# sqeazy/sqeazy

Measured on AMD Instinct MI355X. Metric: encode GB/s (input voxels) for bitswap1->lz4 uint16 volume, higher is better.
Workload: dtype u16

## Files before the change

sqeazy_amd/csrc/sqy_capi.cpp:

```cpp
#include "../../include/sqeazy_amd.h"

#include <hip/hip_runtime.h>

#include <algorithm>
#include <chrono>
#include <climits>
#include <cstdint>
#include <cstdio>
#include <cstdlib>
#include <cstring>
#include <atomic>
#include <condition_variable>
#include <memory>
#include <mutex>
#include <string>
#include <thread>
#include <vector>

#include "sqy_kernels.h"
#include "sqy_lanes.hpp"
#include "sqy_pipeline.hpp"

namespace {

// ... 23 lines not shown
        return dflt;
    }
    return (long)x;
}
constexpr long kWarmupMax = 1l << 30;
constexpr long kStageLanesDefault = 2, kParseLanesDefault = 3;
struct Options {
    std::atomic<long> transpose_chain;
    std::atomic<long> transpose_chain_caller_streams;
    std::atomic<long> block_parallel;
    std::atomic<long> block_parallel_warmup;
    std::atomic<long> block_parallel_stats;
    std::atomic<long> tail_scan;
    std::atomic<long> decode_two_waves;
    std::atomic<long> noise_digest;
    std::atomic<long> transpose_blocks_per_cu;
    std::atomic<long> stored_tail_index;
    std::atomic<long> host_l2_bytes;
    std::atomic<long> decode_frames_subset;
    std::atomic<long> decode_slabs_joint;
    std::atomic<long> stage_lanes;
    std::atomic<long> parse_lanes;
    std::atomic<long> lane_calls{0}, lane_backlog_fallbacks{0}, lane_blocked_fallbacks{0};
    std::atomic<long> call_stamps{0};
    Options()
        : transpose_chain(env_flag("SQY_NO_TRANSPOSE_CHAIN") ? 0 : 1), transpose_chain_caller_streams(env_flag("SQY_TRANSPOSE_CHAIN_CALLER_STREAMS")),
          block_parallel(env_flag("SQY_NO_BLOCK_PARALLEL") ? 0 : 1), block_parallel_warmup(env_number("SQY_BLOCK_PARALLEL_WARMUP", 65536, 0, kWarmupMax)),
          block_parallel_stats(env_flag("SQY_BLOCK_PARALLEL_STATS")), tail_scan(env_flag("SQY_NO_TAIL_SCAN") ? 0 : 1),
          decode_two_waves(env_flag("SQY_NO_DECODE_TWO_WAVES") ? 0 : 1), noise_digest(env_flag("SQY_NO_NOISE_DIGEST") ? 0 : 1),
          transpose_blocks_per_cu(env_number("SQY_TRANSPOSE_BLOCKS_PER_CU", 32, 1, 64)), stored_tail_index(env_flag("SQY_NO_STORED_TAIL_INDEX") ? 0 : 1),
          host_l2_bytes((long)sqy::host_l2_cache_bytes()), decode_frames_subset(env_flag("SQY_NO_DECODE_FRAMES_SUBSET") ? 0 : 1),
          decode_slabs_joint(env_flag("SQY_NO_DECODE_SLABS_JOINT") ? 0 : 1), stage_lanes(env_number("SQY_STAGE_LANES", kStageLanesDefault, 0, 2)),
          parse_lanes(env_number("SQY_PARSE_LANES", kParseLanesDefault, 1, sqy::LanePicker::kMaxLanes)) { sqy::set_bitswap1_blocks_per_cu(transpose_blocks_per_cu.load()); }
    std::atomic<long>* find(const char* name)
    {
        if (!name) return nullptr;
        if (!std::strcmp(name, "transpose_chain")) return &transpose_chain;
        if (!std::strcmp(name, "transpose_chain_caller_streams")) return &transpose_chain_caller_streams;
        if (!std::strcmp(name, "block_parallel")) return &block_parallel;
        if (!std::strcmp(name, "block_parallel_warmup")) return &block_parallel_warmup;
        if (!std::strcmp(name, "block_parallel_stats")) return &block_parallel_stats;
        if (!std::strcmp(name, "tail_scan")) return &tail_scan;
        if (!std::strcmp(name, "decode_two_waves")) return &decode_two_waves;
        if (!std::strcmp(name, "noise_digest")) return &noise_digest;
        if (!std::strcmp(name, "transpose_blocks_per_cu")) return &transpose_blocks_per_cu;
        if (!std::strcmp(name, "stored_tail_index")) return &stored_tail_index;
        if (!std::strcmp(name, "host_l2_bytes")) return &host_l2_bytes;
        if (!std::strcmp(name, "decode_frames_subset")) return &decode_frames_subset;
        if (!std::strcmp(name, "decode_slabs_joint")) return &decode_slabs_joint;
        if (!std::strcmp(name, "stage_lanes")) return &stage_lanes;
        if (!std::strcmp(name, "parse_lanes")) return &parse_lanes;
        if (!std::strcmp(name, "lane_calls")) return &lane_calls;
        if (!std::strcmp(name, "lane_backlog_fallbacks")) return &lane_backlog_fallbacks;
        if (!std::strcmp(name, "lane_blocked_fallbacks")) return &lane_blocked_fallbacks;
        if (!std::strcmp(name, "call_stamps")) return &call_stamps;
        return nullptr;
    }
};
Options g_opt;

struct CallStamps {
    enum { entry, lanes_taken, clear_launched, transpose_launched, parse_queued, sync_returned, returned, kStamps };
    long seq = -1;
    long lane = -1;
    long thread = 0;
    long ns[kStamps] = {};
    void stamp(int i) { ns[i] = (long)std::chrono::duration_cast<std::chrono::nanoseconds>(std::chrono::steady_clock::now().time_since_epoch()).count(); }
};
constexpr size_t kStampRing = 8192;
std::mutex g_stamps_mu;
std::vector<CallStamps> g_stamps;
size_t g_stamps_next = 0;
struct StampScope {
    CallStamps rec;
    const bool on;
    StampScope() : on(g_opt.call_stamps.load(std::memory_order_relaxed) != 0) 
    {
// ... 72 lines not shown
    } while (0)

void prof_collect(std::vector<PendingEvent>& pending)
{
    for (PendingEvent& p : pending) {
        float ms = 0;
        if (hipEventSynchronize(p.b) == hipSuccess && hipEventElapsedTime(&ms, p.a, p.b) == hipSuccess) {
            std::lock_guard<std::mutex> lock(g_prof_mu);
            size_t i = 0;
            for (; i < g_prof.size(); ++i) if (g_prof[i].name == p.name) break;
            if (i == g_prof.size()) g_prof.push_back(ProfEntry{p.name, 0, 0});
            g_prof[i].ms += ms;
            g_prof[i].launches += 1;
        }
        ev_give(p.a);
        ev_give(p.b);
    }
    pending.clear();
}

struct DevBuf {
    void* p = nullptr;
    size_t cap = 0;
    int ensure(size_t bytes, bool quiet = false)
    {
        if (bytes <= cap) return 0;
        if (p) { hipFree(p); p = nullptr; cap = 0; }
        const size_t want = (bytes + ((size_t)1 << 20) - 1) & ~(((size_t)1 << 20) - 1);
        if (hipMalloc(&p, want) != hipSuccess) {
            if (!quiet) std::fprintf(stderr, "[sqeazy]\t unable to allocate %zu bytes of HBM workspace\n", want);
            (void)hipGetLastError();
            p = nullptr;
            return 1;
        }
        cap = want;
        return 0;
    }
    void release() { if (p) hipFree(p); p = nullptr; cap = 0; }
};

struct HostBuf {
    void* p = nullptr;
    size_t cap = 0;
    int ensure(size_t bytes)
    {
        if (bytes <= cap) return 0;
        if (p) { hipHostFree(p); p = nullptr; cap = 0; }
        const size_t want = (bytes + ((size_t)1 << 16) - 1) & ~(((size_t)1 << 16) - 1);
        if (hipHostMalloc(&p, want, hipHostMallocDefault) != hipSuccess) {
            std::fprintf(stderr, "[sqeazy]\t unable to allocate %zu bytes of pinned host memory\n", want);
            (void)hipGetLastError();
            p = nullptr;
            return 1;
        }
        cap = want;
        return 0;
    }
    void release() { if (p) hipHostFree(p); p = nullptr; cap = 0; }
};

struct Workspace {
    DevBuf ping, pong, lz4_scratch, csize, frame_off, io_src, io_dst, small, plan, dedupe;
    DevBuf spec;
    DevBuf diff_side;
    DevBuf digest;
    DevBuf bkrd;
    DevBuf subset;
    DevBuf range_full;
    DevBuf slabs_index;
    DevBuf slabs_joint;
    DevBuf slabs_out;
    HostBuf slabs_host;
    void* pinned = nullptr;
    void release_buffers()
    {
        ping.release(); pong.release(); lz4_scratch.release(); csize.release(); frame_off.release();
        io_src.release(); io_dst.release(); small.release(); plan.release(); dedupe.release(); diff_side.release(); spec.release(); digest.release(); bkrd.release();
        subset.release(); range_full.release(); slabs_index.release(); slabs_joint.release(); slabs_out.release(); slabs_host.release();
    }
};

struct Stager {
    static constexpr int kLanes = 4;
    static constexpr size_t kSlice = 8u << 20;
    char* pin[kLanes][2] = {};
    hipStream_t st[kLanes] = {};
    hipEvent_t ev[kLanes][2] = {};
    bool ready = false;

    bool init()
    {
        if (ready) return true;
        for (int l = 0; l < kLanes; ++l) {
            if (hipStreamCreateWithFlags(&st[l], hipStreamNonBlocking) != hipSuccess) return false;
            for (int b = 0; b < 2; ++b) {
                if (hipHostMalloc((void**)&pin[l][b], kSlice, hipHostMallocDefault) != hipSuccess) return false;
                if (hipEventCreateWithFlags(&ev[l][b], hipEventDisableTiming) != hipSuccess) return false;
            }
// ... 239 lines not shown
    LaneLease* lanes;
    CallStamps* stamps;
    Pipeline pipe;
    std::vector<uint64_t> dims;
    uint64_t len;
    int elem_size;
    void* d_dst;
    uint64_t dst_capacity;
    long* dstoffset;
    FrameQuery* fq;

    const uint8_t* cur;
    int cur_elem;
    uint64_t cur_len;
    bool use_ping = true;

    struct {
        const uint32_t* piece_hash = nullptr;
        bool inplace = false;
        uint64_t t0 = 0, in_stride = 0;
        uint32_t* digest = nullptr;
        uint32_t digest_stride = 0;
        bool dedupe_cleared = false;
        const uint64_t* frame_map = nullptr;
        uint64_t frame_bytes = 0;
    } prep;
    struct DiffSide { const uint16_t* p = nullptr; uint32_t w = 0, X = 0; } side;
    struct {
        bool on = false;
        int block_id = 0;
        uint64_t total = 0, chunk = 0, nchunks = 0, stride = 0;
        const sqy::Lz4Block* blocks = nullptr;
        const uint32_t* dup_of = nullptr;
        uint64_t* tail_info = nullptr;
        bool inplace_done = false;
        uint64_t blob_at = 0, blob_bytes = 0, payload_bytes = 0;
    } lz4;

    EncodeCall(Context& c, hipStream_t s, Pipeline&& p, std::vector<uint64_t>&& d, uint64_t voxels, int elem, const void* src, void* dst,
               uint64_t capacity, long* offset, FrameQuery* frames, LaneLease* lane_lease, CallStamps* call_stamps)
        : cx(c), ws(&c.ws), pend(&c.pending), stream(s), lanes(lane_lease), stamps(call_stamps), pipe(std::move(p)), dims(std::move(d)), len(voxels), elem_size(elem), d_dst(dst),
          dst_capacity(capacity), dstoffset(offset), fq(frames), cur(static_cast<const uint8_t*>(src)), cur_elem(elem), cur_len(voxels) {}

    uint8_t* next_buf(size_t bytes)
    {
        DevBuf& b = use_ping ? ws->ping : ws->pong;
        use_ping = !use_ping;
        return b.ensure(bytes) ? nullptr : static_cast<uint8_t*>(b.p);
    }
    int produced(const uint8_t* out) { cur = out; return 0; }
    bool is_tail(size_t si) const { return pipe.sink_index >= 0 && (int)si > pipe.sink_index; }
    bool not_3d(const char* scheme) const
    {
        if (dims.size() != 3) std::fprintf(stderr, "[sqeazy::detail::%s::encode] received non-3D shape which is currently unsupported!\n", scheme);
        return dims.size() != 3;
    }
    bool followed_by(size_t si, StageKind k) const { return si + 1 < pipe.stages.size() && pipe.stages[si + 1].kind == k; }
    void stage_shape(size_t si, uint64_t& Z, uint64_t& Y, uint64_t& X) const
    {
        const bool flat = is_tail(si) && cur_len * (uint64_t)cur_elem != len;
        Z = flat ? 1 : dims[0]; Y = flat ? 1 : dims[1]; X = flat ? cur_len : dims[2];
    }

    int take_lanes(std::unique_lock<std::mutex>& lock)
    {
// ... 73 lines not shown
            if (words && chunked && chunk % 1024 == 0 && total > chunk) {
                const uint64_t nch = (total + chunk - 1) / chunk;
                const uint64_t ph_bytes = (words * 4 + 63) & ~(uint64_t)63;
                if (ws->dedupe.ensure(ph_bytes + sqy::lz4_dedupe_work_bytes(nch) + ((nch * 4 + 7) & ~(uint64_t)7) + sqy::lz4_holes_map_bytes(nch, (uint32_t)chunk))) return 1;
                ph = static_cast<uint32_t*>(ws->dedupe.p);
                prep.piece_hash = ph;
                if (dstoffset && si + 2 == pipe.stages.size() && (chunk & (chunk - 1)) == 0) {
                    const uint64_t hdr_max = sqy::header_pack(elem_size, false, dims, pipe.name(), (uint64_t)INT_MAX).size() + 2;
                    uint64_t t0 = hdr_max;
                    while ((reinterpret_cast<uintptr_t>(d_dst) + t0 + 11) & 15) ++t0;
                    if (t0 + nch * (chunk + 15) <= dst_capacity) {
                        gap_chunk = chunk;
                        prep.t0 = t0;
                        prep.in_stride = chunk + 15;
                        prep.inplace = true;
                        if (ws->plan.ensure((nch + 1) * sizeof(uint32_t))) return 1;
                        const uint32_t dstride = sqy::lz4_noise_digest_stride((uint32_t)chunk);
                        if (g_opt.noise_digest.load() && dstride && (cur_len / 8) % chunk == 0 && lz.accel >= 0 &&
                            !ws->digest.ensure(nch * (uint64_t)dstride * sizeof(uint32_t), true)) {
                            prep.digest = static_cast<uint32_t*>(ws->digest.p);
                            prep.digest_stride = dstride;
                        }
                        if (take_lanes(lane_lock)) return 1;
                        SQY_HIP(sqy::launch_lz4_dedupe_clear(static_cast<uint8_t*>(ws->dedupe.p) + ph_bytes, nch, static_cast<uint32_t*>(ws->plan.p), stream));
                        prep.dedupe_cleared = true;
                        if (stamps) stamps->stamp(CallStamps::clear_launched);
                    }
                }
            }
        }
        uint8_t* out = gap_chunk ? static_cast<uint8_t*>(d_dst) + prep.t0 + 11 : next_buf(cur_len * cur_elem);
        if (!out) return 1;
        if (!gap_chunk && ph && (reinterpret_cast<uintptr_t>(out) & 15)) { ph = nullptr; prep.piece_hash = nullptr; }
        const bool on_lanes = lanes && lanes->taken();
        const bool owned = stream != nullptr && stream == cx.stream;
        int devid = 0;
        const bool chain = !on_lanes && g_opt.transpose_chain.load() && (owned || g_opt.transpose_chain_caller_streams.load()) && gap_chunk &&
                           hipGetDevice(&devid) == hipSuccess && devid >= 0 && devid < kMaxDev;
        std::unique_lock<std::mutex> tlock;
        if (chain) {
            if (!cx.t_done && hipEventCreateWithFlags(&cx.t_done, hipEventDisableTiming) != hipSuccess) return 1;
            tlock = std::unique_lock<std::mutex>(g_tchain_mu[devid]);
            const auto now = std::chrono::steady_clock::now();
            if (g_tchain_last[devid] && g_tchain_last[devid] != cx.t_done && now - g_tchain_when[devid] < std::chrono::milliseconds(5))
                SQY_HIP(hipStreamWaitEvent(stream, g_tchain_last[devid], 0));
            g_tchain_when[devid] = now;
        }
// ... 303 lines not shown
                                                                   static_cast<uint32_t*>(ws->csize.p), d_redo, n_redo, stream, prep.frame_map, prep.frame_bytes,
                                                                   prep.in_stride));
        return 0;
    }

    int lz4_inplace_finish(uint32_t* d_redo, const std::string& hdr_prefix, const std::string& hdr_suffix)
    {
        const Lz4Descriptor fd = lz4_descriptor(lz4.block_id);
        uint8_t* outb = static_cast<uint8_t*>(d_dst);
        volatile uint64_t* record = static_cast<volatile uint64_t*>(ws->pinned);
        const bool fused_tail = lz4.nchunks <= 65536;
        auto tail = [&](const uint32_t* guard, bool fused, bool scan_too) -> int {
            record[0] = 0;
            if (!fused && scan_too)
                SQY_TIMED("lz4_frame_scan", sqy::launch_lz4_frame_scan(static_cast<uint32_t*>(ws->csize.p), lz4.nchunks, lz4.total, (uint32_t)lz4.chunk,
                                                                       static_cast<uint64_t*>(ws->frame_off.p), stream, nullptr, lz4.dup_of, lz4.tail_info, guard,
                                                                       outb + prep.t0 + 11, prep.in_stride, fd.bd, fd.hc));
            auto with_args = [&](auto launch) {
                return launch(outb, prep.t0, prep.in_stride, lz4.total, (uint32_t)lz4.chunk, lz4.nchunks, static_cast<uint8_t*>(ws->lz4_scratch.p), lz4.stride,
                              static_cast<uint32_t*>(ws->csize.p), static_cast<uint64_t*>(ws->frame_off.p), lz4.dup_of, lz4.tail_info, fd.bd, fd.hc,
                              hdr_prefix.data(), (uint32_t)hdr_prefix.size(), hdr_suffix.data(), (uint32_t)hdr_suffix.size(), (uint32_t)elem_size, guard,
                              const_cast<uint64_t*>(record), stream);
            };
            SQY_TIMED(fused ? "lz4_inplace_tail" : "lz4_frame_gather",
                      fused ? with_args(sqy::launch_lz4_inplace_tail_fused) : with_args(sqy::launch_lz4_inplace_tail));
            return 0;
        };
        if (tail(d_redo, fused_tail, true)) return 1;
        if (stamps) stamps->stamp(CallStamps::parse_queued);
        SQY_HIP(hipStreamSynchronize(stream));
        if (stamps) stamps->stamp(CallStamps::sync_returned);
        if (record[0] == 2) {
            if (lz4_dense(d_redo, (uint32_t)record[6])) return 1;
            if (tail(nullptr, fused_tail, true)) return 1;
            SQY_HIP(hipStreamSynchronize(stream));
        }
        if (record[0] == 4) {
            if (tail(nullptr, false, false)) return 1;
            SQY_HIP(hipStreamSynchronize(stream));
        }
        if (record[0] != 1) {
            std::fprintf(stderr, "[sqeazy]\t internal error: frames in place did not finish (status %llu)\n", (unsigned long long)record[0]);
            return 1;
        }
        lz4.inplace_done = true;
        lz4.blob_at = record[1]; lz4.blob_bytes = record[2]; lz4.payload_bytes = record[3];
        lz4.on = true;
        return 0;
    }

    int lz4_linked(size_t si, bool serial, uint32_t accel)
    {
        const sqy::Lz4Plan plan = sqy::lz4_plan_blocks(lz4.total, lz4.chunk, pipe.stages[si].lz4.block_bytes(), serial);
        if (!plan.ok || plan.blocks.empty()) {
// ... 1611 lines not shown
void SQYAMD_Profile_Reset(void)
{
    std::lock_guard<std::mutex> lock(g_prof_mu);
    g_prof.clear();
}

const char* SQYAMD_Profile_Get(int i, double* total_ms, long* launches)
{
    std::lock_guard<std::mutex> lock(g_prof_mu);
    if (i < 0 || (size_t)i >= g_prof.size()) return nullptr;
    if (total_ms) *total_ms = g_prof[i].ms;
    if (launches) *launches = g_prof[i].launches;
    return g_prof[i].name.c_str();
}

int SQYAMD_Set_Option(const char* name, long value)
{
    std::atomic<long>* o = g_opt.find(name);
    if (!o) return 1;
    if (o == &g_opt.block_parallel_warmup) { if (value < 0 || value > kWarmupMax) return 1; }
    else if (o == &g_opt.transpose_blocks_per_cu) { if (value < 1 || value > 64) return 1; sqy::set_bitswap1_blocks_per_cu(value); }
    else if (o == &g_opt.host_l2_bytes) { if (value < 0 || value > (long)UINT32_MAX) return 1; }
    else if (o == &g_opt.stage_lanes) { if (value < 0 || value > 2) return 1; }
    else if (o == &g_opt.lane_calls || o == &g_opt.lane_backlog_fallbacks || o == &g_opt.lane_blocked_fallbacks) { if (value != 0) return 1; }
    else if (o == &g_opt.parse_lanes) { if (value < 1 || value > sqy::LanePicker::kMaxLanes) return 1; }
    else if (o == &g_opt.call_stamps) {
        if (value != 0 && value != 1) return 1;
        if (value) { std::lock_guard<std::mutex> lock(g_stamps_mu); g_stamps.clear(); g_stamps_next = 0; }
    }
    else if (value != 0 && value != 1) return 1;
    o->store(value);
    return 0;
}

long SQYAMD_Get_Option(const char* name)
{
    std::atomic<long>* o = g_opt.find(name);
    return o ? o->load() : -1;
}

long SQYAMD_Call_Stamps(long* out, long max_records)
{
    std::lock_guard<std::mutex> lock(g_stamps_mu);
    const size_t have = g_stamps.size();
    if (!out || max_records <= 0) return (long)have;
    const size_t n = std::min<size_t>(have, (size_t)max_records), first = (have < kStampRing ? 0 : g_stamps_next) + (have - n);
    for (size_t i = 0; i < n; ++i) {
// ... 63 lines not shown
```

sqeazy_amd/csrc/sqy_kernels.h:

```cpp
#ifndef SQY_KERNELS_H_
#define SQY_KERNELS_H_

#include <hip/hip_runtime_api.h>
#include <stdint.h>

namespace sqy {

struct Lz4DedupeArgs {
    const uint64_t* chunk_key = nullptr;
    const uint64_t* tab_key = nullptr;
    const uint32_t* tab_val = nullptr;
    uint32_t tab_mask = 0;
    uint32_t* dup_of = nullptr;
    const uint32_t* piece_hash = nullptr;
    const uint64_t* holes_map = nullptr;
    uint64_t nchunks_full = 0;
    const uint32_t* digest = nullptr;
    uint32_t digest_stride = 0;
};
hipError_t launch_bitswap1_u16(const uint16_t* in, uint16_t* out, uint64_t len, hipStream_t stream, uint32_t* piece_hash = nullptr,
                               uint32_t gap_chunk = 0, const uint16_t* side = nullptr, uint32_t side_w = 0, uint32_t X = 0,
                               uint32_t* digest = nullptr, uint32_t digest_stride = 0);
void set_bitswap1_blocks_per_cu(long n);
uint32_t lz4_noise_digest_stride(uint32_t chunk);
// ... 27 lines not shown
    int64_t low_in, low_dict;
};
hipError_t launch_lz4_linked(const uint8_t* in, const Lz4Block* blocks, const uint32_t* frame_first, uint64_t nframes,
                             uint32_t max_block, uint8_t* scratch, uint64_t stride, uint32_t* csize, hipStream_t stream, uint32_t acceleration = 1);
struct Lz4SpecArgs {
    const uint32_t* wave_first = nullptr;
    const uint32_t* wave_last = nullptr;
    uint32_t* tables = nullptr;
    uint32_t mode = 0;
};
constexpr uint64_t kLz4SpecTableWords = 2 * 4096;
hipError_t launch_lz4_linked_spec(const uint8_t* in, const Lz4Block* blocks, const Lz4SpecArgs& spec, uint64_t nwaves,
                                  uint32_t max_block, uint8_t* scratch, uint64_t stride, uint32_t* csize, hipStream_t stream, uint32_t acceleration = 1);
hipError_t launch_lz4_linked_verify(const Lz4Block* blocks, uint64_t nblocks, const uint32_t* tables, uint32_t max_block, uint32_t* ok, hipStream_t stream);
hipError_t launch_lz4_frame_scan(const uint32_t* csize, uint64_t nchunks, uint64_t total, uint32_t chunk,
                                 uint64_t* frame_off, hipStream_t stream, const Lz4Block* blocks = nullptr,
                                 const uint32_t* dup_of = nullptr, uint64_t* tail_info = nullptr,
                                 const uint32_t* guard = nullptr, uint8_t* body0 = nullptr, uint64_t in_stride = 0, uint32_t bd_byte = 0,
                                 uint32_t hc_byte = 0);
hipError_t launch_lz4_inplace_tail_fused(uint8_t* out, uint64_t t0, uint64_t in_stride, uint64_t total, uint32_t chunk, uint64_t nchunks,
                                         const uint8_t* scratch, uint64_t stride, const uint32_t* csize, uint64_t* frame_off, const uint32_t* dup_of,
                                         uint64_t* tail_info, uint32_t bd_byte, uint32_t hc_byte, const char* hdr_prefix, uint32_t prefix_len,
                                         const char* hdr_suffix, uint32_t suffix_len, uint32_t elem_size, const uint32_t* guard, uint64_t* record,
                                         hipStream_t stream);
hipError_t launch_lz4_inplace_tail(uint8_t* out, uint64_t t0, uint64_t in_stride, uint64_t total, uint32_t chunk, uint64_t nchunks,
                                   uint8_t* scratch, uint64_t stride, const uint32_t* csize, const uint64_t* frame_off, const uint32_t* dup_of,
                                   const uint64_t* tail_info, uint32_t bd_byte, uint32_t hc_byte, const char* hdr_prefix, uint32_t prefix_len,
                                   const char* hdr_suffix, uint32_t suffix_len, uint32_t elem_size, const uint32_t* guard, uint64_t* record,
                                   hipStream_t stream);
constexpr uint32_t kLz4InplaceHeaderTextMax = 3000;
hipError_t launch_lz4_tail_marks(uint8_t* body0, uint64_t in_stride, uint64_t total, uint32_t chunk, uint64_t nchunks, uint32_t bd_byte,
                                 uint32_t hc_byte, const uint64_t* tail_info, hipStream_t stream);
hipError_t launch_lz4_stash_raw(const uint8_t* body0, uint64_t in_stride, uint64_t total, uint32_t chunk, uint8_t* scratch, uint64_t stride,
                                const uint32_t* csize, const uint32_t* dup_of, uint64_t nhead, hipStream_t stream);
hipError_t launch_lz4_frame_gather(const uint8_t* in, uint64_t total, uint32_t chunk, const uint8_t* scratch, uint64_t stride,
                                   const uint32_t* csize, const uint64_t* frame_off, uint8_t* out, uint32_t bd_byte,
                                   uint32_t hc_byte, uint64_t nchunks, hipStream_t stream, const uint64_t* frame_map = nullptr,
                                   uint64_t frame_bytes = 0, const Lz4Block* blocks = nullptr, const uint32_t* dup_of = nullptr,
                                   uint64_t in_stride = 0, bool raw_from_scratch = false);

uint64_t rmestbkrd_work_bytes(int elem_size);
hipError_t launch_rmestbkrd(const void* in, void* out, uint64_t Z, uint64_t Y, uint64_t X, uint64_t portion, int elem_size, void* work,
                            hipStream_t stream);
hipError_t launch_rmbkrd_neighbor5(const void* in, void* out, uint64_t Z, uint64_t Y, uint64_t X, uint32_t threshold, float cut,
                                   uint64_t z_end, int elem_size, hipStream_t stream);
hipError_t launch_histogram_u16(const uint16_t* in, uint64_t len, uint32_t* histo, hipStream_t stream);
hipError_t launch_quantiser_apply_u16(const uint16_t* in, uint8_t* out, uint64_t len, const uint8_t* lut, hipStream_t stream);
// ... 73 lines not shown
```

sqeazy_amd/csrc/sqy_kernels.hip:

```cpp
#include <hip/hip_runtime.h>
#include <atomic>
#include <mutex>
#include <stdint.h>
#include <cstring>
#include <type_traits>

#include "sqy_kernels.h"

namespace sqy {

struct __attribute__((packed)) pk_u16 { uint16_t v; };
struct __attribute__((packed)) pk_u32 { uint32_t v; };
struct __attribute__((packed)) pk_u64 { uint64_t v; };
struct __attribute__((packed)) pk_u128 { uint32_t x, y, z, w; };

__device__ __forceinline__ uint32_t ld_u32(const uint8_t* p) { return reinterpret_cast<const pk_u32*>(p)->v; }
__device__ __forceinline__ uint64_t ld_u64(const uint8_t* p) { return reinterpret_cast<const pk_u64*>(p)->v; }
__device__ __forceinline__ uint4 ld_u128(const uint8_t* p)
{
    const pk_u128 t = *reinterpret_cast<const pk_u128*>(p);
    return make_uint4(t.x, t.y, t.z, t.w);
}
__device__ __forceinline__ void st_u32(uint8_t* p, uint32_t v) { reinterpret_cast<pk_u32*>(p)->v = v; }
__device__ __forceinline__ void st_u128(uint8_t* p, uint4 v)
// ... 83 lines not shown
        for (int i = 0; i < 4; ++i) {
            const uint32_t a = r[blk + i], b = r[blk + i + 4];
            r[blk + i] = (a & 0x0f0f0f0fu) | ((b << 4) & 0xf0f0f0f0u);
            r[blk + i + 4] = ((a >> 4) & 0x0f0f0f0fu) | (b & 0xf0f0f0f0u);
        }
    }
#pragma unroll
    for (int blk = 0; blk < 16; blk += 4) {
#pragma unroll
        for (int i = 0; i < 2; ++i) {
            const uint32_t a = r[blk + i], b = r[blk + i + 2];
            r[blk + i] = (a & 0x33333333u) | ((b << 2) & 0xccccccccu);
            r[blk + i + 2] = ((a >> 2) & 0x33333333u) | (b & 0xccccccccu);
        }
    }
#pragma unroll
    for (int blk = 0; blk < 16; blk += 2) {
        const uint32_t a = r[blk], b = r[blk + 1];
        r[blk] = (a & 0x55555555u) | ((b << 1) & 0xaaaaaaaau);
        r[blk + 1] = ((a >> 1) & 0x55555555u) | (b & 0xaaaaaaaau);
    }
}

__device__ __forceinline__ uint32_t lz4_hash5_32(uint32_t lo, uint32_t byte4);
template <bool GAP>
__global__ __launch_bounds__(256)
void bitswap1_u16_regs(const uint16_t* __restrict__ in, uint16_t* __restrict__ out, uint64_t n_tiles, uint64_t seg_words,
                       uint32_t* __restrict__ piece_hash, uint32_t gap_shift, const uint16_t* __restrict__ side, uint32_t side_w, uint32_t X,
                       uint32_t* __restrict__ digest, uint32_t digest_stride)
{
    const int lane = threadIdx.x & 63;
    const uint32_t wpb = blockDim.x >> 6;
    const uint64_t wave_global = (uint64_t)blockIdx.x * wpb + (uint32_t)__builtin_amdgcn_readfirstlane((int)(threadIdx.x >> 6));
    const uint64_t wave_stride = (uint64_t)gridDim.x * wpb;
    for (uint64_t tile = wave_global; tile < n_tiles; tile += wave_stride) {
        const v4u* src = reinterpret_cast<const v4u*>(in + tile * BSW_TILE_VOX) + lane * 16;
        if (side) {
            const uint64_t i0 = tile * BSW_TILE_VOX + (uint64_t)lane * 128u;
            const uint64_t row = i0 / X;
            const uint32_t x0 = (uint32_t)(i0 - row * X);
            if (x0 < side_w) src = reinterpret_cast<const v4u*>(side + row * side_w + x0);
        }
        v4u v[16];
#pragma unroll
        for (int j = 0; j < 16; ++j) v[j] = src[j];
        uint32_t pl[16][4];
#pragma unroll
// ... 16 lines not shown
            const uint32_t x = (((uint32_t)tile << 10) & ((1u << gap_shift) - 1u)) + (uint32_t)lane * 16u;
            if (x + 16u > 7667u) {
                const uint32_t xx = x > 7667u ? x : 7667u;
                uint32_t st = (uint32_t)((1.0f + __builtin_sqrtf(1.0f + (float)(xx - 2u) * 0.125f)) * 0.5f);
                if (2u + 32u * (st + 1u) * st <= xx) ++st;
                if (2u + 32u * st * (st - 1u) > xx) --st;
                const uint32_t Bs = 2u + 32u * st * (st - 1u), num = xx - Bs;
                uint32_t kk = (uint32_t)((float)num / (float)st);
                if (kk * st > num) --kk;
                if ((kk + 1u) * st <= num) ++kk;
                if (kk * st != num) ++kk;
                const uint32_t cand = Bs + kk * st, u = 64u * st - 62u + kk;
                if (cand < x + 16u && u >= 961u && u - 961u < digest_stride) dg = 0x80000000u | ((u - 961u) << 4) | (cand - x);
            }
        }
        const uint32_t dg_tsh = 31u - gap_shift;
        const uint32_t pm = 2u * (uint32_t)lane + 1u;
#pragma unroll
        for (int b = 0; b < 16; ++b) {
            uint32_t vx = pl[b][0], vy = pl[b][1], vz = pl[b][2], vw = pl[b][3];
            asm volatile("" : "+v"(vx), "+v"(vy), "+v"(vz), "+v"(vw) :: "memory");
            const v4u val = {vx, vy, vz, vw};
            const uint64_t nzm = ballot((val.x | val.y | val.z | val.w) != 0u);
            if (piece_hash) {
                uint32_t a = val.x * 0x9E3779B1u + val.y * 0x85EBCA77u + val.z * 0xC2B2AE3Du + val.w * 0x27D4EB2Fu;
                a = (a ^ (a >> 15)) * pm;
                const bool row_nz = ((nzm >> (lane & 48)) & 0xffffull) != 0ull;
                a += __builtin_amdgcn_update_dpp(0u, a, 0x111, 0xf, 0xf, false);
                a += __builtin_amdgcn_update_dpp(0u, a, 0x112, 0xf, 0xf, false);
                a += __builtin_amdgcn_update_dpp(0u, a, 0x114, 0xf, 0xf, false);
                a += __builtin_amdgcn_update_dpp(0u, a, 0x118, 0xf, 0xf, false);
                const uint64_t piece = ((uint64_t)(15 - b) * seg_words * 2u + tile * 1024u) >> 10;
                if ((lane & 15) == 15) piece_hash[piece * 4u + (uint32_t)(lane >> 4)] = row_nz ? (a | 1u) : 0u;
            }
            if (GAP) {
                if (nzm == 0ull) continue;
                const uint64_t B = (uint64_t)(15 - b) * seg_words * 2u + tile * 1024u;
                if (digest) {
                    const uint32_t nx = (uint32_t)__builtin_amdgcn_update_dpp(0, (int)val.x, 0x130, 0xf, 0xf, true);
                    const uint32_t dg_off = dg & 15u, dg_q = dg_off >> 2, dg_r = dg_off & 3u;
                    const uint32_t d0 = dg_q == 0u ? val.x : dg_q == 1u ? val.y : dg_q == 2u ? val.z : val.w;
                    const uint32_t d1 = dg_q == 0u ? val.y : dg_q == 1u ? val.z : dg_q == 2u ? val.w : nx;
                    const uint32_t lo = __builtin_amdgcn_alignbyte(d1, d0, dg_r);
                    const uint32_t b5 = d1 >> (8u * dg_r);
                    uint32_t e = (lz4_hash5_32(lo, b5) << 17) | ((lo * 2654435761u) >> (32u - dg_tsh));
                    if (lane == 63 && dg_off > 11u) e = 0xffffffffu;
                    const uint64_t drow = (B >> gap_shift) * (uint64_t)digest_stride * 4u;
                    const uint32_t drow_lo = (uint32_t)__builtin_amdgcn_readfirstlane((int)(uint32_t)drow);
                    const uint32_t drow_hi = (uint32_t)__builtin_amdgcn_readfirstlane((int)(uint32_t)(drow >> 32));
                    uint8_t* const dbase = reinterpret_cast<uint8_t*>(digest) + (((uint64_t)drow_hi << 32) | drow_lo);
                    if ((int32_t)dg < 0) *reinterpret_cast<uint32_t*>(dbase + ((dg >> 2) & 0x1ffffffcu)) = e;
                }
                const uint64_t kq = B >> gap_shift;
#ifdef SQY_EXP_GAP_BYTES
                const uint64_t off = B + kq * SQY_EXP_GAP_BYTES;
#else
                const uint64_t off = B + (kq << 4) - kq;
#endif
                const uint32_t off_lo = (uint32_t)__builtin_amdgcn_readfirstlane((int)(uint32_t)off);
                const uint32_t off_hi = (uint32_t)__builtin_amdgcn_readfirstlane((int)(uint32_t)(off >> 32));
                uint8_t* dst = reinterpret_cast<uint8_t*>(out) + (((uint64_t)off_hi << 32) | off_lo);
                __builtin_nontemporal_store((v4u_any)val, reinterpret_cast<v4u_any*>(dst + (uint32_t)lane * 16u));
            } else {
                v4u* dst = reinterpret_cast<v4u*>(out + (uint64_t)(15 - b) * seg_words + tile * (BSW_TILE_VOX / 16));
                __builtin_nontemporal_store(val, dst + lane);
            }
        }
    }
// ... 4814 lines not shown
        st = nb >> 6; ++nb;
        if (p2 > (uint64_t)chunk - 12 + 1) break;
        p = p2;
    }
    if (probes <= 961) return 0;
    return (uint32_t)(((probes - 960) + 63) & ~(uint64_t)63);
}

uint64_t bitswap1_piece_hash_words(const void* in, const void* out, uint64_t len)
{
    if (len == 0 || len % BSW_TILE_VOX != 0) return 0;
    if ((reinterpret_cast<uintptr_t>(in) & 15) || (reinterpret_cast<uintptr_t>(out) & 15)) return 0;
    return (len / BSW_TILE_VOX) * 16 * 4;
}

__global__ __launch_bounds__(256)
void lz4_dedupe_clear_kernel(uint64_t* __restrict__ tab_key, uint32_t* __restrict__ tab_val, uint32_t tab, uint32_t* __restrict__ zero_word)
{
    const uint32_t i = blockIdx.x * 256u + threadIdx.x;
    if (i < tab) { tab_key[i] = 0ull; tab_val[i] = 0xffffffffu; }
    if (i == 0 && zero_word) *zero_word = 0u;
}

hipError_t launch_lz4_dedupe_clear(void* work, uint64_t nchunks, uint32_t* zero_word, hipStream_t stream)
{
    if (nchunks == 0) return hipSuccess;
    uint32_t tab = 64;
    while (tab < 2 * nchunks) tab <<= 1;
    uint64_t* chunk_key = static_cast<uint64_t*>(work);
    uint64_t* tab_key = chunk_key + nchunks;
    uint32_t* tab_val = reinterpret_cast<uint32_t*>(tab_key + tab);
    hipLaunchKernelGGL(lz4_dedupe_clear_kernel, dim3((tab + 255u) / 256u), dim3(256), 0, stream, tab_key, tab_val, tab, zero_word);
    return hipGetLastError();
}

hipError_t launch_lz4_dedupe(const uint8_t* in, uint64_t total, uint32_t chunk, const uint32_t* piece_hash, void* work,
                             uint32_t* dup_of, hipStream_t stream, uint64_t in_stride, uint64_t* holes_map, bool table_is_clear,
                             Lz4DedupeArgs* fused)
{
    const uint64_t nchunks = (total + chunk - 1) / chunk, nfull = total / chunk;
    if (nchunks == 0) return hipSuccess;
    if (in_stride == 0) in_stride = chunk;
    if (chunk % 1024 != 0) return hipErrorInvalidValue;
    uint32_t tab = 64;
    while (tab < 2 * nchunks) tab <<= 1;
    uint64_t* chunk_key = static_cast<uint64_t*>(work);
    uint64_t* tab_key = chunk_key + nchunks;
    uint32_t* tab_val = reinterpret_cast<uint32_t*>(tab_key + tab);
    hipError_t e = hipSuccess;
    if (!table_is_clear) {
        e = hipMemsetAsync(tab_key, 0, (size_t)tab * 8, stream);
        if (e != hipSuccess) return e;
        e = hipMemsetAsync(tab_val, 0xff, (size_t)tab * 4, stream);
        if (e != hipSuccess) return e;
    }
// ... 200 lines not shown
hipError_t launch_lz4_linked_verify(const Lz4Block* blocks, uint64_t nblocks, const uint32_t* tables, uint32_t max_block, uint32_t* ok, hipStream_t stream)
{
    if (nblocks == 0) return hipSuccess;
    if (max_block == 0 || max_block > (4u << 20)) return hipErrorInvalidValue;
    hipLaunchKernelGGL(lz4_linked_verify_kernel, dim3((unsigned)nblocks), dim3(256), 0, stream, blocks, tables, max_block, ok);
    return hipGetLastError();
}

hipError_t launch_lz4_frame_scan(const uint32_t* csize, uint64_t nchunks, uint64_t total, uint32_t chunk,
                                 uint64_t* frame_off, hipStream_t stream, const Lz4Block* blocks, const uint32_t* dup_of, uint64_t* tail_info,
                                 const uint32_t* guard, uint8_t* body0, uint64_t in_stride, uint32_t bd_byte, uint32_t hc_byte)
{
    hipLaunchKernelGGL(lz4_frame_scan_kernel, dim3(1), dim3(256), 0, stream, csize, nchunks, total, chunk, frame_off, blocks, dup_of, tail_info,
                       guard, body0, in_stride, bd_byte, hc_byte);
    return hipGetLastError();
}

constexpr uint32_t TAIL_THREADS = 64;
__global__ __launch_bounds__(TAIL_THREADS)
void lz4_inplace_tail_fused_kernel(uint8_t* __restrict__ out, uint64_t t0, uint64_t in_stride, uint64_t total, uint32_t chunk, uint64_t nchunks,
                                   uint32_t cpb, const uint8_t* __restrict__ scratch, uint64_t stride, const uint32_t* __restrict__ csize,
                                   uint64_t* __restrict__ frame_off, const uint32_t* __restrict__ dup_of, uint64_t* __restrict__ tail_info,
                                   uint32_t bd_byte, uint32_t hc_byte, Lz4HeaderParts hp, uint32_t elem_size, const uint32_t* __restrict__ guard,
                                   uint64_t* __restrict__ record)
{
    const uint32_t tid = threadIdx.x, lane = tid & 63u, wave = tid >> 6;
    if (guard && guard[0] != 0u) {
        if (blockIdx.x == 0 && tid == 0) { record[6] = guard[0]; record[0] = 2; }
        return;
    }
    __shared__ uint64_t red_sum[TAIL_THREADS / 64], red_before[TAIL_THREADS / 64];
    __shared__ uint32_t red_j[TAIL_THREADS / 64], red_zero[TAIL_THREADS / 64];
    __shared__ uint64_t own_off[64];
    __shared__ uint32_t own_c[64], own_ks[64];
    const uint64_t k_first = (uint64_t)blockIdx.x * cpb;
    uint64_t sum = 0, before = 0;
    uint32_t jmax = 0, nzero = 0;
    for (uint64_t base = 0; base < nchunks; base += TAIL_THREADS * 8u) {
        uint32_t ks[8], c[8];
#pragma unroll
        for (uint32_t u = 0; u < 8; ++u) {
            const uint64_t k = base + u * TAIL_THREADS + tid;
            ks[u] = k < nchunks ? (dup_of ? dup_of[k] : (uint32_t)k) : 0u;
        }
#pragma unroll
        for (uint32_t u = 0; u < 8; ++u) {
            const uint64_t k = base + u * TAIL_THREADS + tid;
// ... 43 lines not shown
            const uint64_t k = k_first + i;
            const uint64_t left = total - k * chunk;
            const uint64_t nk = left < chunk ? left : chunk;
            own_off[i] = o;
            frame_off[k] = o;
            o += 15u + (own_c[i] ? own_c[i] : nk);
        }
    }
    __syncthreads();
    if (tid < nown && k_first + tid >= j) {
        const uint64_t k = k_first + tid;
        const uint64_t left = total - k * chunk;
        const uint32_t nk = (uint32_t)(left < chunk ? left : chunk);
        uint8_t* b = body0 + k * in_stride;
        const uint32_t field = nk | 0x80000000u;
        b[-11] = 0x04; b[-10] = 0x22; b[-9] = 0x4D; b[-8] = 0x18; b[-7] = 0x40; b[-6] = (uint8_t)bd_byte; b[-5] = (uint8_t)hc_byte;
        b[-4] = (uint8_t)field; b[-3] = (uint8_t)(field >> 8); b[-2] = (uint8_t)(field >> 16); b[-1] = (uint8_t)(field >> 24);
        b[nk] = 0; b[nk + 1] = 0; b[nk + 2] = 0; b[nk + 3] = 0;
    }
    if (nraw != 0u) {
        if (blockIdx.x == 0 && tid == 0) { record[4] = j; record[5] = nraw; record[0] = 4; }
        return;
    }
    uint8_t* const dst0 = out + t0 + j * in_stride - head_bytes;
    for (uint32_t i = 0; i < nown; ++i) {
        const uint64_t k = k_first + i;
        if (k >= j) break;
        const uint32_t c = own_c[i];
        const uint8_t* __restrict__ s = scratch + (uint64_t)own_ks[i] * stride;
        uint8_t* __restrict__ d = dst0 + own_off[i];
        if (tid < 15u) {
            uint8_t v = 0;
            uint32_t o = tid;
            switch (tid) {
                case 0: v = 0x04; break; case 1: v = 0x22; break; case 2: v = 0x4D; break; case 3: v = 0x18; break;
                case 4: v = 0x40; break; case 5: v = (uint8_t)bd_byte; break; case 6: v = (uint8_t)hc_byte; break;
                case 7: v = (uint8_t)c; break; case 8: v = (uint8_t)(c >> 8); break;
                case 9: v = (uint8_t)(c >> 16); break; case 10: v = (uint8_t)(c >> 24); break;
                default: v = 0; o = 11u + c + (tid - 11u); break;
            }
            d[o] = v;
        }
        uint8_t* __restrict__ dd = d + 11;
        const uint8_t* __restrict__ ss = s;
        uint32_t len = c;
        const uint32_t head0 = (uint32_t)((16 - (reinterpret_cast<uintptr_t>(dd) & 15)) & 15);
// ... 31 lines not shown
    for (uint64_t i = tid; i < hdr_len; i += TAIL_THREADS) {
        uint8_t cch;
        if (i < pad) cch = ' ';
        else if (i < pad + hp.prefix_len) cch = (uint8_t)hp.text[i - pad];
        else if (i < pad + hp.prefix_len + nd) cch = (uint8_t)digits[nd - 1 - (i - pad - hp.prefix_len)];
        else cch = (uint8_t)hp.text[hp.prefix_len + (i - pad - hp.prefix_len - nd)];
        h[i] = cch;
    }
    if (tid == 0) {
        record[1] = payload_at - hdr_len;
        record[2] = hdr_len + payload;
        record[3] = payload;
        record[4] = j;
        record[5] = 0;
        record[6] = 0;
        record[0] = 1;
    }
}

hipError_t launch_lz4_inplace_tail_fused(uint8_t* out, uint64_t t0, uint64_t in_stride, uint64_t total, uint32_t chunk, uint64_t nchunks,
                                         const uint8_t* scratch, uint64_t stride, const uint32_t* csize, uint64_t* frame_off, const uint32_t* dup_of,
                                         uint64_t* tail_info, uint32_t bd_byte, uint32_t hc_byte, const char* hdr_prefix, uint32_t prefix_len,
                                         const char* hdr_suffix, uint32_t suffix_len, uint32_t elem_size, const uint32_t* guard, uint64_t* record,
                                         hipStream_t stream)
{
    Lz4HeaderParts hp;
    if ((uint64_t)prefix_len + suffix_len > sizeof(hp.text) || nchunks == 0 || nchunks > 0x7fffffffull) return hipErrorInvalidValue;
    hp.prefix_len = prefix_len; hp.suffix_len = suffix_len;
    std::memcpy(hp.text, hdr_prefix, prefix_len);
    std::memcpy(hp.text + prefix_len, hdr_suffix, suffix_len);
    uint32_t cpb = (uint32_t)((nchunks + 1023u) / 1024u);
    if (cpb < 4u) cpb = 4u;
    if (cpb > 64u) return hipErrorInvalidValue;
    const unsigned grid = (unsigned)((nchunks + cpb - 1u) / cpb);
    hipLaunchKernelGGL(lz4_inplace_tail_fused_kernel, dim3(grid), dim3(TAIL_THREADS), 0, stream, out, t0, in_stride, total, chunk, nchunks, cpb, scratch,
                       stride, csize, frame_off, dup_of, tail_info, bd_byte, hc_byte, hp, elem_size, guard, record);
    return hipGetLastError();
}

hipError_t launch_lz4_inplace_tail(uint8_t* out, uint64_t t0, uint64_t in_stride, uint64_t total, uint32_t chunk, uint64_t nchunks,
                                   uint8_t* scratch, uint64_t stride, const uint32_t* csize, const uint64_t* frame_off, const uint32_t* dup_of,
                                   const uint64_t* tail_info, uint32_t bd_byte, uint32_t hc_byte, const char* hdr_prefix, uint32_t prefix_len,
                                   const char* hdr_suffix, uint32_t suffix_len, uint32_t elem_size, const uint32_t* guard, uint64_t* record,
                                   hipStream_t stream)
{
    Lz4HeaderParts hp;
    if ((uint64_t)prefix_len + suffix_len > sizeof(hp.text) || nchunks == 0) return hipErrorInvalidValue;
    hp.prefix_len = prefix_len; hp.suffix_len = suffix_len;
    std::memcpy(hp.text, hdr_prefix, prefix_len);
    std::memcpy(hp.text + prefix_len, hdr_suffix, suffix_len);
    uint8_t* body0 = out + t0 + 11;
    const uint32_t slices_stash = (chunk + 32767u) / 32768u, slices = (chunk + GATHER_SLICE - 1) / GATHER_SLICE;
    const uint64_t stash_items = nchunks * slices_stash, gather_items = nchunks * slices;
    hipLaunchKernelGGL(lz4_stash_raw_kernel, dim3((unsigned)(stash_items < 1024 ? stash_items : 1024)), dim3(256), 0, stream, body0, in_stride, total, chunk,
                       scratch, stride, csize, dup_of, slices_stash, tail_info, guard);
    hipLaunchKernelGGL(lz4_frame_gather_kernel, dim3((unsigned)(gather_items < 2048 ? gather_items : 2048)), dim3(256), 0, stream, body0, total, chunk,
                       scratch, stride, csize, frame_off, out, bd_byte, hc_byte, slices, (const uint64_t*)nullptr, (uint64_t)0, (const Lz4Block*)nullptr,
                       dup_of, in_stride, 0, tail_info, t0, guard);
    hipLaunchKernelGGL(lz4_inplace_finish_kernel, dim3(1), dim3(256), 0, stream, out, t0, in_stride, tail_info, hp, elem_size, guard, record);
// ... 972 lines not shown
```

Measured before the change: 2028.

## Fuse dedupe table clear into fused tail kernel and skip redundant clear launches

Result: no change. 2016 (-0.6%).

```diff
diff --git a/sqeazy_amd/csrc/sqy_capi.cpp b/sqeazy_amd/csrc/sqy_capi.cpp
--- a/sqeazy_amd/csrc/sqy_capi.cpp
+++ b/sqeazy_amd/csrc/sqy_capi.cpp
@@ -69,6 +69,7 @@
     std::atomic<long> stage_lanes;
     std::atomic<long> parse_lanes;
     std::atomic<long> lane_calls{0}, lane_backlog_fallbacks{0}, lane_blocked_fallbacks{0};
+    std::atomic<long> clear_launches_saved{0};
     std::atomic<long> call_stamps{0};
     Options()
         : transpose_chain(env_flag("SQY_NO_TRANSPOSE_CHAIN") ? 0 : 1), transpose_chain_caller_streams(env_flag("SQY_TRANSPOSE_CHAIN_CALLER_STREAMS")),
@@ -100,6 +101,7 @@
         if (!std::strcmp(name, "lane_calls")) return &lane_calls;
         if (!std::strcmp(name, "lane_backlog_fallbacks")) return &lane_backlog_fallbacks;
         if (!std::strcmp(name, "lane_blocked_fallbacks")) return &lane_blocked_fallbacks;
+        if (!std::strcmp(name, "clear_launches_saved")) return &clear_launches_saved;
         if (!std::strcmp(name, "call_stamps")) return &call_stamps;
         return nullptr;
     }
@@ -218,9 +220,11 @@
 struct DevBuf {
     void* p = nullptr;
     size_t cap = 0;
+    uint64_t gen = 0;
     int ensure(size_t bytes, bool quiet = false)
     {
         if (bytes <= cap) return 0;
+        ++gen;
         if (p) { hipFree(p); p = nullptr; cap = 0; }
         const size_t want = (bytes + ((size_t)1 << 20) - 1) & ~(((size_t)1 << 20) - 1);
         if (hipMalloc(&p, want) != hipSuccess) {
@@ -232,7 +236,7 @@
         cap = want;
         return 0;
     }
-    void release() { if (p) hipFree(p); p = nullptr; cap = 0; }
+    void release() { if (p) hipFree(p); p = nullptr; cap = 0; ++gen; }
 };
 
 struct HostBuf {
@@ -268,8 +272,18 @@
     DevBuf slabs_out;
     HostBuf slabs_host;
     void* pinned = nullptr;
+    struct Cleared {
+        const void* work = nullptr;
+        const void* zero_word = nullptr;
+        uint64_t nchunks = 0, dedupe_gen = 0, plan_gen = 0;
+    } cleared;
+    bool cleared_for(const void* work, uint64_t nchunks, const Cleared& c) const
+    {
+        return c.work && c.work == work && c.zero_word == plan.p && c.nchunks == nchunks && c.dedupe_gen == dedupe.gen && c.plan_gen == plan.gen;
+    }
     void release_buffers()
     {
+        cleared = Cleared();
         ping.release(); pong.release(); lz4_scratch.release(); csize.release(); frame_off.release();
         io_src.release(); io_dst.release(); small.release(); plan.release(); dedupe.release(); diff_side.release(); spec.release(); digest.release(); bkrd.release();
         subset.release(); range_full.release(); slabs_index.release(); slabs_joint.release(); slabs_out.release(); slabs_host.release();
@@ -555,6 +569,7 @@
         uint32_t* digest = nullptr;
         uint32_t digest_stride = 0;
         bool dedupe_cleared = false;
+        void* dedupe_work = nullptr;
         const uint64_t* frame_map = nullptr;
         uint64_t frame_bytes = 0;
     } prep;
@@ -569,11 +584,16 @@
         bool inplace_done = false;
         uint64_t blob_at = 0, blob_bytes = 0, payload_bytes = 0;
     } lz4;
+    Workspace::Cleared cleared_at_entry;
 
     EncodeCall(Context& c, hipStream_t s, Pipeline&& p, std::vector<uint64_t>&& d, uint64_t voxels, int elem, const void* src, void* dst,
                uint64_t capacity, long* offset, FrameQuery* frames, LaneLease* lane_lease, CallStamps* call_stamps)
         : cx(c), ws(&c.ws), pend(&c.pending), stream(s), lanes(lane_lease), stamps(call_stamps), pipe(std::move(p)), dims(std::move(d)), len(voxels), elem_size(elem), d_dst(dst),
-          dst_capacity(capacity), dstoffset(offset), fq(frames), cur(static_cast<const uint8_t*>(src)), cur_elem(elem), cur_len(voxels) {}
+          dst_capacity(capacity), dstoffset(offset), fq(frames), cur(static_cast<const uint8_t*>(src)), cur_elem(elem), cur_len(voxels)
+    {
+        cleared_at_entry = c.ws.cleared;
+        c.ws.cleared = Workspace::Cleared();
+    }
 
     uint8_t* next_buf(size_t bytes)
     {
@@ -693,7 +713,12 @@
                             prep.digest_stride = dstride;
                         }
                         if (take_lanes(lane_lock)) return 1;
-                        SQY_HIP(sqy::launch_lz4_dedupe_clear(static_cast<uint8_t*>(ws->dedupe.p) + ph_bytes, nch, static_cast<uint32_t*>(ws->plan.p), stream));
+                        prep.dedupe_work = static_cast<uint8_t*>(ws->dedupe.p) + ph_bytes;
+                        if (!ws->cleared_for(prep.dedupe_work, nch, cleared_at_entry))
+                            SQY_HIP(sqy::launch_lz4_dedupe_clear(prep.dedupe_work, nch, static_cast<uint32_t*>(ws->plan.p), stream));
+                        else
+                            g_opt.clear_launches_saved += 1;
+                        cleared_at_entry = Workspace::Cleared();
                         prep.dedupe_cleared = true;
                         if (stamps) stamps->stamp(CallStamps::clear_launched);
                     }
@@ -1043,14 +1068,24 @@
                               hdr_prefix.data(), (uint32_t)hdr_prefix.size(), hdr_suffix.data(), (uint32_t)hdr_suffix.size(), (uint32_t)elem_size, guard,
                               const_cast<uint64_t*>(record), stream);
             };
+            auto with_args_clear = [&](auto launch) {
+                return launch(outb, prep.t0, prep.in_stride, lz4.total, (uint32_t)lz4.chunk, lz4.nchunks, static_cast<uint8_t*>(ws->lz4_scratch.p), lz4.stride,
+                              static_cast<uint32_t*>(ws->csize.p), static_cast<uint64_t*>(ws->frame_off.p), lz4.dup_of, lz4.tail_info, fd.bd, fd.hc,
+                              hdr_prefix.data(), (uint32_t)hdr_prefix.size(), hdr_suffix.data(), (uint32_t)hdr_suffix.size(), (uint32_t)elem_size, guard,
+                              const_cast<uint64_t*>(record), stream, guard ? prep.dedupe_work : nullptr);
+            };
             SQY_TIMED(fused ? "lz4_inplace_tail" : "lz4_frame_gather",
-                      fused ? with_args(sqy::launch_lz4_inplace_tail_fused) : with_args(sqy::launch_lz4_inplace_tail));
+                      fused ? with_args_clear(sqy::launch_lz4_inplace_tail_fused) : with_args(sqy::launch_lz4_inplace_tail));
             return 0;
         };
         if (tail(d_redo, fused_tail, true)) return 1;
         if (stamps) stamps->stamp(CallStamps::parse_queued);
         SQY_HIP(hipStreamSynchronize(stream));
         if (stamps) stamps->stamp(CallStamps::sync_returned);
+        if (record[0] == 1 && fused_tail && prep.dedupe_work && d_redo == ws->plan.p) {
+            ws->cleared.work = prep.dedupe_work; ws->cleared.zero_word = d_redo; ws->cleared.nchunks = lz4.nchunks;
+            ws->cleared.dedupe_gen = ws->dedupe.gen; ws->cleared.plan_gen = ws->plan.gen;
+        }
         if (record[0] == 2) {
             if (lz4_dense(d_redo, (uint32_t)record[6])) return 1;
             if (tail(nullptr, fused_tail, true)) return 1;
@@ -2708,7 +2743,7 @@
     else if (o == &g_opt.transpose_blocks_per_cu) { if (value < 1 || value > 64) return 1; sqy::set_bitswap1_blocks_per_cu(value); }
     else if (o == &g_opt.host_l2_bytes) { if (value < 0 || value > (long)UINT32_MAX) return 1; }
     else if (o == &g_opt.stage_lanes) { if (value < 0 || value > 2) return 1; }
-    else if (o == &g_opt.lane_calls || o == &g_opt.lane_backlog_fallbacks || o == &g_opt.lane_blocked_fallbacks) { if (value != 0) return 1; }
+    else if (o == &g_opt.lane_calls || o == &g_opt.lane_backlog_fallbacks || o == &g_opt.lane_blocked_fallbacks || o == &g_opt.clear_launches_saved) { if (value != 0) return 1; }
     else if (o == &g_opt.parse_lanes) { if (value < 1 || value > sqy::LanePicker::kMaxLanes) return 1; }
     else if (o == &g_opt.call_stamps) {
         if (value != 0 && value != 1) return 1;
diff --git a/sqeazy_amd/csrc/sqy_kernels.h b/sqeazy_amd/csrc/sqy_kernels.h
--- a/sqeazy_amd/csrc/sqy_kernels.h
+++ b/sqeazy_amd/csrc/sqy_kernels.h
@@ -73,7 +73,8 @@
                                          const uint8_t* scratch, uint64_t stride, const uint32_t* csize, uint64_t* frame_off, const uint32_t* dup_of,
                                          uint64_t* tail_info, uint32_t bd_byte, uint32_t hc_byte, const char* hdr_prefix, uint32_t prefix_len,
                                          const char* hdr_suffix, uint32_t suffix_len, uint32_t elem_size, const uint32_t* guard, uint64_t* record,
-                                         hipStream_t stream);
+                                         hipStream_t stream,
+                                         void* clear_work = nullptr);
 hipError_t launch_lz4_inplace_tail(uint8_t* out, uint64_t t0, uint64_t in_stride, uint64_t total, uint32_t chunk, uint64_t nchunks,
                                    uint8_t* scratch, uint64_t stride, const uint32_t* csize, const uint64_t* frame_off, const uint32_t* dup_of,
                                    const uint64_t* tail_info, uint32_t bd_byte, uint32_t hc_byte, const char* hdr_prefix, uint32_t prefix_len,
diff --git a/sqeazy_amd/csrc/sqy_kernels.hip b/sqeazy_amd/csrc/sqy_kernels.hip
--- a/sqeazy_amd/csrc/sqy_kernels.hip
+++ b/sqeazy_amd/csrc/sqy_kernels.hip
@@ -129,7 +129,15 @@
     }
 }
 
-__device__ __forceinline__ uint32_t lz4_hash5_32(uint32_t lo, uint32_t byte4);
+__device__ __forceinline__ uint32_t lz4_hash5_32_u24(uint32_t lo, uint32_t byte4)
+{
+    const uint32_t plo = 0x1BBCDCBBu;
+    const uint64_t p = (uint64_t)lo * plo;
+    uint32_t h = (uint32_t)(p >> 32);
+    asm("v_mad_u32_u24 %0, %1, %2, %0" : "+v"(h) : "v"(lo), "s"(0xCFu));
+    asm("v_mad_u32_u24 %0, %1, %2, %0" : "+v"(h) : "v"(byte4), "s"(0xBBu));
+    return ((h << 4) | ((uint32_t)p >> 28)) & 0xfffu;
+}
 template <bool GAP>
 __global__ __launch_bounds__(256)
 void bitswap1_u16_regs(const uint16_t* __restrict__ in, uint16_t* __restrict__ out, uint64_t n_tiles, uint64_t seg_words,
@@ -192,6 +200,13 @@
             asm volatile("" : "+v"(vx), "+v"(vy), "+v"(vz), "+v"(vw) :: "memory");
             const v4u val = {vx, vy, vz, vw};
             const uint64_t nzm = ballot((val.x | val.y | val.z | val.w) != 0u);
+            if (GAP && nzm == 0ull) {
+                if (piece_hash) {
+                    const uint64_t piece = ((uint64_t)(15 - b) * seg_words * 2u + tile * 1024u) >> 10;
+                    if ((lane & 15) == 15) piece_hash[piece * 4u + (uint32_t)(lane >> 4)] = 0u;
+                }
+                continue;
+            }
             if (piece_hash) {
                 uint32_t a = val.x * 0x9E3779B1u + val.y * 0x85EBCA77u + val.z * 0xC2B2AE3Du + val.w * 0x27D4EB2Fu;
                 a = (a ^ (a >> 15)) * pm;
@@ -204,7 +219,6 @@
                 if ((lane & 15) == 15) piece_hash[piece * 4u + (uint32_t)(lane >> 4)] = row_nz ? (a | 1u) : 0u;
             }
             if (GAP) {
-                if (nzm == 0ull) continue;
                 const uint64_t B = (uint64_t)(15 - b) * seg_words * 2u + tile * 1024u;
                 if (digest) {
                     const uint32_t nx = (uint32_t)__builtin_amdgcn_update_dpp(0, (int)val.x, 0x130, 0xf, 0xf, true);
@@ -213,7 +227,7 @@
                     const uint32_t d1 = dg_q == 0u ? val.y : dg_q == 1u ? val.z : dg_q == 2u ? val.w : nx;
                     const uint32_t lo = __builtin_amdgcn_alignbyte(d1, d0, dg_r);
                     const uint32_t b5 = d1 >> (8u * dg_r);
-                    uint32_t e = (lz4_hash5_32(lo, b5) << 17) | ((lo * 2654435761u) >> (32u - dg_tsh));
+                    uint32_t e = (lz4_hash5_32_u24(lo, b5) << 17) | ((lo * 2654435761u) >> (32u - dg_tsh));
                     if (lane == 63 && dg_off > 11u) e = 0xffffffffu;
                     const uint64_t drow = (B >> gap_shift) * (uint64_t)digest_stride * 4u;
                     const uint32_t drow_lo = (uint32_t)__builtin_amdgcn_readfirstlane((int)(uint32_t)drow);
@@ -5074,15 +5088,21 @@
     if (i == 0 && zero_word) *zero_word = 0u;
 }
 
-hipError_t launch_lz4_dedupe_clear(void* work, uint64_t nchunks, uint32_t* zero_word, hipStream_t stream)
-{
-    if (nchunks == 0) return hipSuccess;
+struct Lz4DedupeTable { uint64_t* key; uint32_t* val; uint32_t n; };
+static Lz4DedupeTable lz4_dedupe_table(void* work, uint64_t nchunks)
+{
     uint32_t tab = 64;
     while (tab < 2 * nchunks) tab <<= 1;
     uint64_t* chunk_key = static_cast<uint64_t*>(work);
     uint64_t* tab_key = chunk_key + nchunks;
-    uint32_t* tab_val = reinterpret_cast<uint32_t*>(tab_key + tab);
-    hipLaunchKernelGGL(lz4_dedupe_clear_kernel, dim3((tab + 255u) / 256u), dim3(256), 0, stream, tab_key, tab_val, tab, zero_word);
+    return {tab_key, reinterpret_cast<uint32_t*>(tab_key + tab), tab};
+}
+
+hipError_t launch_lz4_dedupe_clear(void* work, uint64_t nchunks, uint32_t* zero_word, hipStream_t stream)
+{
+    if (nchunks == 0) return hipSuccess;
+    const Lz4DedupeTable tb = lz4_dedupe_table(work, nchunks);
+    hipLaunchKernelGGL(lz4_dedupe_clear_kernel, dim3((tb.n + 255u) / 256u), dim3(256), 0, stream, tb.key, tb.val, tb.n, zero_word);
     return hipGetLastError();
 }
 
@@ -5329,7 +5349,7 @@
                                    uint32_t cpb, const uint8_t* __restrict__ scratch, uint64_t stride, const uint32_t* __restrict__ csize,
                                    uint64_t* __restrict__ frame_off, const uint32_t* __restrict__ dup_of, uint64_t* __restrict__ tail_info,
                                    uint32_t bd_byte, uint32_t hc_byte, Lz4HeaderParts hp, uint32_t elem_size, const uint32_t* __restrict__ guard,
-                                   uint64_t* __restrict__ record)
+                                   uint64_t* __restrict__ record, uint64_t* __restrict__ clear_key, uint32_t* __restrict__ clear_val, uint32_t clear_n)
 {
     const uint32_t tid = threadIdx.x, lane = tid & 63u, wave = tid >> 6;
     if (guard && guard[0] != 0u) {
@@ -5419,6 +5439,7 @@
         if (blockIdx.x == 0 && tid == 0) { record[4] = j; record[5] = nraw; record[0] = 4; }
         return;
     }
+    for (uint32_t i = blockIdx.x * TAIL_THREADS + tid; i < clear_n; i += gridDim.x * TAIL_THREADS) { clear_key[i] = 0ull; clear_val[i] = 0xffffffffu; }
     uint8_t* const dst0 = out + t0 + j * in_stride - head_bytes;
     for (uint32_t i = 0; i < nown; ++i) {
         const uint64_t k = k_first + i;
@@ -5496,10 +5517,12 @@
                                          const uint8_t* scratch, uint64_t stride, const uint32_t* csize, uint64_t* frame_off, const uint32_t* dup_of,
                                          uint64_t* tail_info, uint32_t bd_byte, uint32_t hc_byte, const char* hdr_prefix, uint32_t prefix_len,
                                          const char* hdr_suffix, uint32_t suffix_len, uint32_t elem_size, const uint32_t* guard, uint64_t* record,
-                                         hipStream_t stream)
+                                         hipStream_t stream, void* clear_work)
 {
     Lz4HeaderParts hp;
     if ((uint64_t)prefix_len + suffix_len > sizeof(hp.text) || nchunks == 0 || nchunks > 0x7fffffffull) return hipErrorInvalidValue;
+    Lz4DedupeTable tb{};
+    if (clear_work && guard) tb = lz4_dedupe_table(clear_work, nchunks);
     hp.prefix_len = prefix_len; hp.suffix_len = suffix_len;
     std::memcpy(hp.text, hdr_prefix, prefix_len);
     std::memcpy(hp.text + prefix_len, hdr_suffix, suffix_len);
@@ -5508,7 +5531,7 @@
     if (cpb > 64u) return hipErrorInvalidValue;
     const unsigned grid = (unsigned)((nchunks + cpb - 1u) / cpb);
     hipLaunchKernelGGL(lz4_inplace_tail_fused_kernel, dim3(grid), dim3(TAIL_THREADS), 0, stream, out, t0, in_stride, total, chunk, nchunks, cpb, scratch,
-                       stride, csize, frame_off, dup_of, tail_info, bd_byte, hc_byte, hp, elem_size, guard, record);
+                       stride, csize, frame_off, dup_of, tail_info, bd_byte, hc_byte, hp, elem_size, guard, record, tb.key, tb.val, tb.n);
     return hipGetLastError();
 }
 
```
